# Ladme/groan_rs

Hardware: AMD Instinct MI355X
Metric: frames/sec RMSD-fit, 1e6 atoms triclinic, 1/2/4/8 GPUs; HBM GB/s vs peak (higher is better)
Workload: dtype f32 (fp64 accumulators)

## Files before the change

### groan_rs_amd/csrc/gr_api.hip

```cpp
#include <hip/hip_runtime.h>

#include <cmath>
#include <cstdio>
#include <cstdlib>
#include <cstring>
#include <map>
#include <string>
#include <vector>

#include "../../include/groan_hip.h"
#include "gr_batch.h"
#include "gr_buf.h"
#include "gr_workers.h"
#include "gr_container.h"
#include "gr_kernels.h"
#include "gr_hot.h"
#include "gr_resident.h"
#include "gr_small.h"
#include "gr_xtc.h"
#include "gr_shape.h"
#include "gr_xtc_dev.h"
#include "gr_xtc_enc_dev.h"
#include "gr_trr.h"
#include "gr_cellgrid.h"
// ... 394 lines not shown
    if (c->in_flight && slot < c->in_flight_s0 + c->in_flight_n && c->in_flight_s0 < slot + n)
        return fail(c, GR_E_INVALID_ARG, "upload into a slot of the batch in flight: call gr_rmsd_batch_end first (or use the other half of the double buffer)");
    return GR_OK;
}

struct SlotUse {
    gr_ctx *c; uint32_t first, n;
    bool quiet = false;
    SlotUse(gr_ctx *ctx, uint32_t first_slot, uint32_t count = 1) : c(ctx), first(first_slot), n(count) {
        for (uint32_t s = first; s < first + n && s < c->n_slots; ++s)
            if (c->upload_pending[s]) { (void)hipStreamWaitEvent(c->stream, c->ev_ready[s], 0); c->upload_pending[s] = 0; }
    }
    ~SlotUse() {
        if (quiet) return;
        const uint64_t gen = ++c->done_gen;
        (void)hipEventRecord(c->ev_done_ring[gen % 64], c->stream);
        for (uint32_t s = first; s < first + n && s < c->n_slots; ++s) c->slot_gen[s] = gen;
    }
};

static hipError_t sync_ingest(gr_ctx *c) {
    hipError_t e = hipStreamSynchronize(c->copy_stream);
    if (e == hipSuccess && c->unpack_stream) e = hipStreamSynchronize(c->unpack_stream);
    return e;
}
static int slot_box_wait(gr_ctx *c, uint32_t slot) {
    if (c->ev_ready[slot]) HIPCHK(c, hipEventSynchronize(c->ev_ready[slot]));
    else HIPCHK(c, hipEventCreateWithFlags(&c->ev_ready[slot], hipEventDisableTiming));
    return GR_OK;
}
void box_fill(gr_ctx *c, uint32_t slot, const float *box9) {
    GrBox &b = c->boxes_host[slot];
    if (!box9) {
        gr_box_setup(nullptr, &b);
        c->box_status[slot] = GR_E_NO_BOX; c->box9_set[slot] = 0;
    } else {
        const int ok = gr_box_setup(box9, &b);
        memcpy(&c->box9_host[9 * (size_t)slot], box9, 9 * sizeof(float));
        c->box9_set[slot] = 1;
        if (!ok) c->box_status[slot] = GR_E_ZERO_BOX;
        else if (b.ncand > GR_MAX_CAND) c->box_status[slot] = GR_E_UNSUPPORTED_BOX;
        else c->box_status[slot] = GR_OK;
    }
}
int set_box(gr_ctx *c, uint32_t slot, const float *box9, hipStream_t on = nullptr) {
    box_fill(c, slot, box9);
    HIPCHK(c, hipMemcpyAsync(c->boxes_dev + slot, &c->boxes_host[slot], sizeof(GrBox), hipMemcpyHostToDevice, on ? on : c->stream));
    return GR_OK;
}

int set_boxes_same(gr_ctx *c, uint32_t first_slot, uint32_t n, const float *box9, hipStream_t on = nullptr) {
    if (n == 0) return GR_OK;
    float keep[9];
    if (box9) memcpy(keep, box9, sizeof keep);
    box_fill(c, first_slot, box9 ? keep : nullptr);
    for (uint32_t f = 1; f < n; ++f) {
        const uint32_t s = first_slot + f;
        c->boxes_host[s] = c->boxes_host[first_slot];
        c->box_status[s] = c->box_status[first_slot]; c->box9_set[s] = c->box9_set[first_slot];
        if (box9) memcpy(&c->box9_host[9 * (size_t)s], keep, sizeof keep);
    }
    HIPCHK(c, hipMemcpyAsync(c->boxes_dev + first_slot, c->boxes_host + first_slot, (size_t)n * sizeof(GrBox), hipMemcpyHostToDevice, on ? on : c->stream));
    return GR_OK;
}

int ensure_staging(gr_ctx *c, float **buf) {
    if (*buf) return GR_OK;
    HIPCHK(c, hipMalloc(buf, c->frame_stride * sizeof(float)));
    HIPCHK(c, hipMemsetAsync(*buf, 0, c->frame_stride * sizeof(float), c->stream));
    HIPCHK(c, hipStreamSynchronize(c->stream));
    return GR_OK;
}
int untile_slot(gr_ctx *c, uint32_t slot) {
    int st = ensure_staging(c, &c->aos_dl); if (st) return st;
    const uint32_t ng = (uint32_t)(c->n_pad >> 2);
    k_untile<<<dim3((ng + 255) / 256), dim3(256), 0, c->stream>>>(c->frames + (size_t)slot * c->frame_stride, c->aos_dl, ng);
    HIPCHK(c, hipGetLastError());
    return GR_OK;
}

int ensure_event(gr_ctx *c, hipEvent_t *ev, bool timing) {
    if (*ev) return GR_OK;
    HIPCHK(c, timing ? hipEventCreate(ev) : hipEventCreateWithFlags(ev, hipEventDisableTiming));
    return GR_OK;
}
#define EVREC(ctx, ev, timing, stream) do { int s_ = ensure_event((ctx), &(ev), (timing)); if (s_) return s_; HIPCHK((ctx), hipEventRecord((ev), (stream))); } while (0)

int state_reset(gr_ctx *c, uint32_t n) {
    k_state_reset<<<dim3((n + 63) / 64), dim3(64), 0, c->stream>>>(c->state_dev, n);
    HIPCHK(c, hipGetLastError());
    return GR_OK;
}

int fetch_states(gr_ctx *c, uint32_t n) {
    HIPCHK(c, hipMemcpyAsync(c->state_host, c->state_dev, n * sizeof(GrFrameState), hipMemcpyDeviceToHost, c->stream));
    HIPCHK(c, hipStreamSynchronize(c->stream));
    return GR_OK;
}

int frame_status(gr_ctx *c, const GrFrameState &st) {
    if (st.status == GR_OK) return GR_OK;
    if (st.status == GR_E_NO_POSITION) return fail(c, GR_E_NO_POSITION, "atom has no position", st.err_index);
    if (st.status == GR_E_NO_MASS) return fail(c, GR_E_NO_MASS, "atom has no mass", st.err_index);
    return fail(c, st.status, "frame analysis failed");
}

static bool small_ok(const gr_ctx *c, const GrSel &sel) { return c->small_max != 0 && c->small_state != nullptr && sel.n <= c->small_max && !c->profile; }
static int small_wait(gr_ctx *c, uint32_t seq, uint32_t words = 1) {
    volatile uint32_t *w = c->small_flag;
    const auto t0 = std::chrono::steady_clock::now();
    for (uint32_t spins = 0; w[0] != seq || w[words - 1] != seq; ++spins) {
        if ((spins & 1023u) == 1023u && std::chrono::steady_clock::now() - t0 > std::chrono::milliseconds(20)) {
            c->small_sync_fallbacks++;
            HIPCHK(c, hipStreamSynchronize(c->stream));
            if (w[0] != seq || w[words - 1] != seq) return fail(c, GR_E_HIP, "a single-wave kernel ended without publishing its result");
            break;
        }
    }
    std::atomic_thread_fence(std::memory_order_acquire);
    c->small_calls++;
    return GR_OK;
}

static int res_next_epoch(gr_ctx *c, uint32_t *epoch) {
    if (++c->res_epoch == 0u) {
        HIPCHK(c, hipStreamSynchronize(c->stream));
        if (c->res_wgrec.get()) HIPCHK(c, hipMemset(c->res_wgrec.get(), 0, c->res_wgrec.cap() * sizeof(unsigned long long)));
        HIPCHK(c, hipMemset(c->res_rec, 0, (size_t)GR_MAX_BATCH * 16 * sizeof(unsigned long long)));
        HIPCHK(c, hipMemset(c->res_abort + 2, 0, 2 * sizeof(uint32_t)));
        c->res_epoch = 1u;
    }
    *epoch = c->res_epoch;
    return GR_OK;
}
static int res_wgrec_reserve(gr_ctx *c, size_t rec_words, hipStream_t S) {
    bool grew = false;
    HIPCHK(c, c->res_wgrec.reserve(rec_words, grbuf::exact, &grew));
    const hipError_t e = grew ? hipMemsetAsync(c->res_wgrec.get(), 0, rec_words * sizeof(unsigned long long), S) : hipSuccess;
    if (e != hipSuccess) c->res_wgrec.release();
    HIPCHK(c, e);
    return GR_OK;
}
static int res_test_no_start(gr_ctx *c, uint32_t epoch) {
    if (!c->res_test_no_start) return GR_OK;
    const unsigned long long two = 2ull | ((unsigned long long)epoch << 32);
    c->res_test_no_start = 0;
    HIPCHK(c, hipMemcpyAsync(c->res_abort + 2, &two, sizeof two, hipMemcpyHostToDevice, c->stream));
    HIPCHK(c, hipStreamSynchronize(c->stream));
    return GR_OK;
}
template <int MODE>
static int res_close(gr_ctx *c, uint32_t nb, const double *fit_partials, uint32_t nparts, double sum_w, uint32_t epoch, bool fresh, uint32_t *seq) {
    const uint32_t sq = c->res_seq + 1u;
    k_res_close<MODE><<<dim3(nb), dim3(64), 0, c->stream>>>(fit_partials, nparts, sum_w, c->state_dev, c->res_rec, epoch, fresh ? 1u : 0u, c->res_abort, c->res_closed + nb,
                                                        c->res_out_dev->st, c->res_out_dev->words, &c->res_out_dev->seq, sq);
    HIPCHK(c, hipGetLastError());
    c->res_seq = sq; c->res_closed += nb; *seq = sq;
    return GR_OK;
}
static int res_collect(gr_ctx *c, uint32_t seq, uint32_t nb, uint32_t epoch, bool *started) {
    volatile uint32_t *w = &c->res_out->seq;
    const auto t0 = std::chrono::steady_clock::now();
    for (uint32_t spins = 0; *w != seq; ++spins) {
        if ((spins & 1023u) == 1023u && std::chrono::steady_clock::now() - t0 > std::chrono::milliseconds(20)) {
            c->res_sync_fallbacks++;
            HIPCHK(c, hipStreamSynchronize(c->stream));
            if (*w != seq) return fail(c, GR_E_HIP, "the kernel behind the resident pass ended without publishing its results");
            break;
        }
    }
    std::atomic_thread_fence(std::memory_order_acquire);
    memcpy(c->state_host, c->res_out->st, (size_t)nb * sizeof(GrFrameState));
    memcpy(c->res_words_host, c->res_out->words, 12 * sizeof(uint32_t));
    for (int k = 0; k < 2; ++k) { const uint32_t v = c->res_words_host[8 + k]; c->res_words_host[8 + k] = v - c->res_late_seen[k]; c->res_late_seen[k] = v; }
    *started = c->res_words_host[2] == 1u && c->res_words_host[3] == epoch;
    if (!*started || c->res_words_host[0]) HIPCHK(c, hipStreamSynchronize(c->stream));
    return GR_OK;
}

int center_stage(gr_ctx *c, uint32_t first_slot, uint32_t nf, const GrSel &sel, int kind, int weighted,
                 int mass_first, int target, int only_status = 0) {
    if (small_ok(c, sel)) {
        k_center_small_stage<<<dim3(nf), dim3(64), 0, c->stream>>>(c->frames, c->frame_stride, first_slot, c->masses, sel, c->boxes_dev, kind, weighted, mass_first, target, c->state_dev, only_status);
        HIPCHK(c, hipGetLastError());
        return GR_OK;
    }
    uint32_t nch = chunks_for(sel);
    if (nf > 1 && nch >= 8) nch &= ~7u;
    const dim3 grid(nch, nf), wg(GR_WG);
    if (kind == 0) k_center_sums<0><<<grid, wg, 0, c->stream>>>(c->frames, c->frame_stride, first_slot, c->masses, sel, c->boxes_dev, c->state_dev, weighted, c->cen_partials, only_status);
    else if (kind == 1) k_center_sums<1><<<grid, wg, 0, c->stream>>>(c->frames, c->frame_stride, first_slot, c->masses, sel, c->boxes_dev, c->state_dev, weighted, c->cen_partials, only_status);
    else k_center_sums<2><<<grid, wg, 0, c->stream>>>(c->frames, c->frame_stride, first_slot, c->masses, sel, c->boxes_dev, c->state_dev, weighted, c->cen_partials, only_status);
    k_center_finalize<<<dim3(nf), dim3(GR_WG), 0, c->stream>>>(c->cen_partials, nch, c->boxes_dev, first_slot, kind, weighted, mass_first, target, sel.n, c->state_dev, only_status);
    HIPCHK(c, hipGetLastError());
    return GR_OK;
}

int pbc_center_stages(gr_ctx *c, uint32_t first_slot, uint32_t nf, const GrSel &sel, int weighted, int only_status = 0) {
    if (small_ok(c, sel) && only_status == 0) {
        k_center_small_pbc<<<dim3(nf), dim3(64), 0, c->stream>>>(c->frames, c->frame_stride, first_slot, c->masses, sel, c->boxes_dev, weighted, c->state_dev);
        HIPCHK(c, hipGetLastError());
        return GR_OK;
    }
    int st = center_stage(c, first_slot, nf, sel, 1, 0, 0, 0, only_status);
    if (st != GR_OK) return st;
    return center_stage(c, first_slot, nf, sel, 2, weighted, 0, 1, only_status);
}

static bool center_onepass_ok(const gr_ctx *c, const GrSel &sel) {
    return c->com_onepass_min != 0 && (sel.contiguous || sel.masked) && sel.n >= c->com_onepass_min && c->two_pass;
}
static int pbc_center_onepass(gr_ctx *c, uint32_t s0, uint32_t nb, const GrSel &sel, int weighted) {
    GrPlanDev plan; memset(&plan, 0, sizeof plan);
    plan.w_is_mass = weighted ? 1u : 0u;
    plan.n = sel.n; plan.sw = 1.0;
    const uint32_t nch = batch_chunks(c, sel, nb);
    if (sel.masked) {
        k_sums_pk<true, false, true><<<dim3(nch, nb), dim3(GR_WG), 0, c->stream>>>(c->frames, c->frame_stride, s0, c->masses, sel, c->boxes_dev, plan, c->acc_partials,
                                                                                   c->fuse ? c->fuse_cnt : nullptr, c->fuse ? c->state_dev : nullptr);
        if (!c->fuse) k_rmsd_finalize_lite<true><<<dim3(nb), dim3(64), 0, c->stream>>>(c->acc_partials, nch, c->frames, c->frame_stride, s0, sel, c->boxes_dev, plan, c->state_dev);
    } else if (c->fuse) {
        k_sums_pk<true><<<dim3(nch, nb), dim3(GR_WG), 0, c->stream>>>(c->frames, c->frame_stride, s0, c->masses, sel, c->boxes_dev, plan, c->acc_partials, c->fuse_cnt, c->state_dev);
    } else {
        k_sums_pk<true><<<dim3(nch, nb), dim3(GR_WG), 0, c->stream>>>(c->frames, c->frame_stride, s0, c->masses, sel, c->boxes_dev, plan, c->acc_partials, nullptr, nullptr);
        k_rmsd_finalize_lite<true><<<dim3(nb), dim3(64), 0, c->stream>>>(c->acc_partials, nch, c->frames, c->frame_stride, s0, sel, c->boxes_dev, plan, c->state_dev);
    }
    HIPCHK(c, hipGetLastError());
    return GR_OK;
}
static int center_redo_fallbacks(gr_ctx *c, uint32_t s0, uint32_t nb, const GrSel &sel, int weighted, std::vector<GrFrameState> &res) {
    uint32_t n_fb = 0, n_amb = 0;
    for (uint32_t f = 0; f < nb; ++f) { n_fb += c->state_host[f].status == GR_ST_FALLBACK; n_amb += c->state_host[f].status == GR_ST_AMBIG; }
    if (n_fb || n_amb) {
        c->center_fallbacks += n_fb + n_amb;
        int st = GR_OK;
        if (n_amb) { st = center_stage(c, s0, nb, sel, 1, 0, 0, 0, GR_ST_AMBIG); if (st) return st; }
        if (n_fb) { st = pbc_center_stages(c, s0, nb, sel, weighted, GR_ST_FALLBACK); if (st) return st; }
        st = fetch_states(c, nb); if (st) return st;
    }
    res.assign(c->state_host, c->state_host + nb);
    return GR_OK;
}

}

static int gr_abi_guard() { return GR_E_HIP; }

extern "C" {

const char *gr_version(void) { return "groan_hip 0.1.0 (gfx950)"; }

const char *gr_status_string(int s) try {
    switch (s) {
    case GR_OK: return "ok";
    case GR_E_NO_BOX: return "simulation box does not exist";
    case GR_E_NOT_ORTHOGONAL: return "simulation box is not orthogonal";
    case GR_E_ZERO_BOX: return "box length is zero or negative";
    case GR_E_EMPTY_GROUP: return "group is empty";
    case GR_E_INCONSISTENT_GROUP: return "group has a different number of atoms in reference and target";
    case GR_E_NO_POSITION: return "atom has undefined position";
    case GR_E_NO_MASS: return "atom has undefined mass";
    case GR_E_GROUP_NOT_FOUND: return "group does not exist";
    case GR_E_OUT_OF_RANGE: return "atom index out of range";
    case GR_E_INVALID_ARG: return "invalid argument";
    case GR_E_GROUP_EXISTS: return "group already existed and was overwritten";
    case GR_E_HIP: return "HIP runtime error";
    case GR_E_NO_DEVICE: return "no usable HIP device";
    case GR_E_UNSUPPORTED_BOX: return "box too skewed for the minimum-image table";
    case GR_E_IO: return "file could not be opened or read";
    case GR_E_FORMAT: return "not a valid xtc file";
    case GR_E_INVALID_NAME: return "invalid group name";
    case GR_E_EMPTY_CHAIN: return "no acceptor and no donor atoms detected for chain";
    case GR_E_NONEXISTENT_CHAIN: return "chain does not exist";
    case GR_E_DUPLICATE_PAIR: return "pair of chains requested multiple times";
    case GR_E_UNUSED_CHAIN: return "not all chains are used";
    case GR_E_INVALID_BOND: return "invalid bond";
    case GR_E_INVALID_SPAN: return "invalid span of the grid map";
    case GR_E_INVALID_TILE: return "invalid grid tile";
    default: return "unknown status";
    }
} catch (...) { return nullptr; }

int gr_device_count(int *count) try {
    int n = 0;
    if (hipGetDeviceCount(&n) != hipSuccess) { if (count) *count = 0; return GR_E_NO_DEVICE; }
    if (count) *count = n;
    return n > 0 ? GR_OK : GR_E_NO_DEVICE;
} catch (...) { return gr_abi_guard(); }

gr_ctx *gr_ctx_create(int device, uint64_t n_atoms, uint32_t n_slots, int *status) try {
    int dummy; if (!status) status = &dummy;
    int ndev = 0;
    if (hipGetDeviceCount(&ndev) != hipSuccess || ndev <= 0 || device < 0 || device >= ndev) { *status = GR_E_NO_DEVICE; return nullptr; }
    if (n_atoms == 0 || n_atoms > 0xFFFFFFF0ull || n_slots == 0) { *status = GR_E_INVALID_ARG; return nullptr; }
    if (hipSetDevice(device) != hipSuccess) { *status = GR_E_NO_DEVICE; return nullptr; }
    gr_ctx *c = new gr_ctx();
    c->device = device; c->n = n_atoms; c->n_pad = (n_atoms + 255) & ~255ull; c->n_slots = n_slots;
    c->frame_stride = (size_t)c->n_pad * 3;
    bool ok = true;
    ok = ok && hipStreamCreateWithFlags(&c->stream, hipStreamNonBlocking) == hipSuccess;
    ok = ok && hipStreamCreateWithFlags(&c->copy_stream, hipStreamNonBlocking) == hipSuccess;
    for (int k = 0; k < 64; ++k) ok = ok && hipEventCreateWithFlags(&c->ev_done_ring[k], hipEventDisableTiming) == hipSuccess;
    c->ev_ready.assign(n_slots, nullptr); c->upload_pending.assign(n_slots, 0); c->slot_gen.assign(n_slots, 0);
    ok = ok && hipMalloc(&c->fuse_cnt, 2 * GR_MAX_BATCH * sizeof(uint32_t)) == hipSuccess;
    ok = ok && hipMemset(c->fuse_cnt, 0, 2 * GR_MAX_BATCH * sizeof(uint32_t)) == hipSuccess;
    { hipDeviceProp_t prop; if (hipGetDeviceProperties(&prop, device) == hipSuccess) c->n_cus = (uint32_t)prop.multiProcessorCount; }
    ok = ok && hipMalloc(&c->frames, (size_t)n_slots * c->frame_stride * sizeof(float)) == hipSuccess;
    ok = ok && hipMalloc(&c->masses, c->n_pad * sizeof(float)) == hipSuccess;
// ... 2625 lines not shown
```

### groan_rs_amd/csrc/gr_resident.h

```cpp
#pragma once
#include <type_traits>
#include "gr_hot.h"

struct GrResShape {
    static constexpr int LANES = 512, WAVES = LANES / 64;
#ifndef GR_RES_K
#define GR_RES_K 6
#endif
    static constexpr int K = GR_RES_K;
    static constexpr int R = 8;
    static constexpr int PARK_F4 = K * 3 * LANES;
    static constexpr int WSUM_F = R * WAVES * 32;
#ifdef GR_EXP_TIMELINE
    static constexpr int TL_BYTES = 128 * 4 * 8;
#else
    static constexpr int TL_BYTES = 0;
#endif
    static constexpr int LDS_BYTES = PARK_F4 * 16 + WSUM_F * 4 + R * WAVES * 8 + 3 * R * 4 + 2 * WAVES * 4 + TL_BYTES;
    static constexpr int REC_PER_WAVE = 256 / WAVES, LANES_PER_REC = 64 / REC_PER_WAVE, WORDS_PER_LANE = 32 / LANES_PER_REC;
};
#ifndef GR_RES_SLEEP
#define GR_RES_SLEEP 2
#endif
#ifndef GR_RES_BAL
// ... 792 lines not shown
            }
        } else if (status == 0) {
            GrResRot T;
            T.r00 = rec.r00; T.r10 = rec.r10; T.r20 = rec.r20; T.r01 = rec.r01; T.r11 = rec.r11; T.r21 = rec.r21;
            T.r02 = rec.r02; T.r12 = rec.r12; T.r22 = rec.r22;
            if (V) {
                const float t0x = rec.t0x, t0y = rec.t0y, t0z = rec.t0z;
                T.sx = T.sy = T.sz = 0.f;
                fit_group_v(GA, ra, T, t0x, t0y, t0z, oa, rs);
                if (GB.valid) fit_group_v(GB, rb, T, t0x, t0y, t0z, ob, rs);
            } else {
                T.sx = rec.sx; T.sy = rec.sy; T.sz = rec.sz;
                const GrBox *boxp = boxes + first_slot + kf(j);
                gr_res_fit_group<WMASS>(GA, ra.r0, ra.r1, ra.r2, T, B, boxp, cx, cy, cz, oa.r0, oa.r1, oa.r2, rs);
                if (GB.valid) gr_res_fit_group<WMASS>(GB, rb.r0, rb.r1, rb.r2, T, B, boxp, cx, cy, cz, ob.r0, ob.r1, ob.r2, rs);
            }
        }
        {
#ifdef GR_EXP_NOSTORE
            const __amdgpu_buffer_rsrc_t out = gr_buf_rsrc(frames + (size_t)(first_slot + kf(j)) * frame_stride, 0u);
#else
            const __amdgpu_buffer_rsrc_t out = gr_buf_rsrc(frames + (size_t)(first_slot + kf(j)) * frame_stride, status == 0 ? slot_bytes : 0u);
#endif
            gr_buf_store_stream(out, offA, oa.r0); gr_buf_store_stream(out, offA + 1024u, oa.r1); gr_buf_store_stream(out, offA + 2048u, oa.r2);
            gr_buf_store_stream(out, offB, ob.r0); gr_buf_store_stream(out, offB + 1024u, ob.r1); gr_buf_store_stream(out, offB + 2048u, ob.r2);
        }
        n_fitted = j + 1u;
        if (MODE == 1) return;
        const float wtot = gr_wave_allsum_f32(rs);
        if (lane == 0) fit_partials[((size_t)kf(j) * ctl.wgs_frame + wg) * WAVES + wave] = (double)wtot;
    };

    Landing L0, L1;
    L0.a.r0 = L0.a.r1 = L0.a.r2 = L0.b.r0 = L0.b.r1 = L0.b.r2 = zero4; L0.gx = L0.gy = L0.gz = 0.f;
    L1 = L0;
    Rows Q0, Q1, Q2, Q3, Q4, Q5;
    Q0.r0 = Q0.r1 = Q0.r2 = zero4; Q1 = Q0; Q2 = Q0; Q3 = Q0; Q4 = Q0; Q5 = Q0;
    unsigned long long rv = 0ull;
    gate(0);
    if (n_turns) request(0, L0);
    const uint32_t n_iter = n_turns + K;
    const GrBoxU B0 = gr_box_uniform(boxes + first_slot);
    auto lds_put = [&](uint32_t slot, const Rows &rw) { park[(slot * 3 + 0) * LANES + tid] = rw.r0; park[(slot * 3 + 1) * LANES + tid] = rw.r1; park[(slot * 3 + 2) * LANES + tid] = rw.r2; };
    auto lds_get = [&](uint32_t slot) { Rows rw; rw.r0 = park[(slot * 3 + 0) * LANES + tid]; rw.r1 = park[(slot * 3 + 1) * LANES + tid]; rw.r2 = park[(slot * 3 + 2) * LANES + tid]; return rw; };
    auto step_sums_first = [&](uint32_t i, Landing &cur, Landing &nxt) {
        rv = request_rec(i >= K && i < n_iter ? i - K : 0u);
#ifdef GR_EXP_NOLOAD
        if (i < 2) request(i + 1, nxt);
#else
        GR_STEP_STAMP(6);
        gate(i + 1);
        GR_STEP_STAMP(0);
        request(i + 1, nxt);
#endif
        balance(i);
        const GrBoxU Bf = UBOX ? B0 : gr_box_uniform(boxes + first_slot + kf(i >= K ? i - K : 0u));
        const GrBoxU Bs = UBOX ? B0 : gr_box_uniform(boxes + first_slot + kf(i < n_turns ? i : 0u));
        Rows va = cur.a, vb = cur.b;
        const uint32_t ps = i % K;
        GR_STEP_STAMP(1);
        if (i < n_turns) { if constexpr (MODE == 1) sums_cen(i, cur, Bs); else sums(i, cur, Bs, va, vb); }
#if GR_RES_LATE_COMBINE
        if (i == n_turns && n_turns > 0u && claim(n_turns - 1u)) { if constexpr (MODE == 1) combine_cen(n_turns - 1u); else combine_rmsd(n_turns - 1u); }
#endif
        GR_STEP_STAMP(3);
        if (i >= K) {
            Rows qb;
            if (ps == 0u) { qb = Q0; asm volatile("; set 0 out"); } else if (ps == 1u) { qb = Q1; asm volatile("; set 1 out"); } else if (ps == 2u) { qb = Q2; asm volatile("; set 2 out"); }
            else if (ps == 3u) { qb = Q3; asm volatile("; set 3 out"); } else if (ps == 4u) { qb = Q4; asm volatile("; set 4 out"); } else { qb = Q5; asm volatile("; set 5 out"); }
            fit(i - K, rv, lds_get(ps), qb, Bf);
            if (bail) return;
        }
        GR_STEP_STAMP(5);
        if (i < n_turns) {
            lds_put(ps, va);
            if (ps == 0u) { Q0 = vb; asm volatile("; set 0 in"); } else if (ps == 1u) { Q1 = vb; asm volatile("; set 1 in"); } else if (ps == 2u) { Q2 = vb; asm volatile("; set 2 in"); }
            else if (ps == 3u) { Q3 = vb; asm volatile("; set 3 in"); } else if (ps == 4u) { Q4 = vb; asm volatile("; set 4 in"); } else { Q5 = vb; asm volatile("; set 5 in"); }
        }
    };
    auto step_fit_first = [&](uint32_t i, Landing &cur, Landing &nxt) {
#ifdef GR_EXP_NOLOAD
        if (i < 2) request(i + 1, nxt);
#elif !defined(GR_EXP_LATE_REQUEST)
        gate(i + 1);
        request(i + 1, nxt);
#endif
        balance(i);
        const GrBoxU Bf = UBOX ? B0 : gr_box_uniform(boxes + first_slot + kf(i >= K ? i - K : 0u));
        const GrBoxU Bs = UBOX ? B0 : gr_box_uniform(boxes + first_slot + kf(i < n_turns ? i : 0u));
        Rows va = cur.a, vb = cur.b;
        const uint32_t ps = i % K;
        if (i >= K) {
            Rows qb;
            if (ps == 0u) { qb = Q0; asm volatile("; set 0 out"); } else if (ps == 1u) { qb = Q1; asm volatile("; set 1 out"); } else if (ps == 2u) { qb = Q2; asm volatile("; set 2 out"); }
            else if (ps == 3u) { qb = Q3; asm volatile("; set 3 out"); } else if (ps == 4u) { qb = Q4; asm volatile("; set 4 out"); } else { qb = Q5; asm volatile("; set 5 out"); }
            fit(i - K, rv, lds_get(ps), qb, Bf);
            if (bail) return;
        }
        rv = request_rec(i + 1 >= K && i + 1 < n_iter ? i + 1 - K : 0u);
#ifdef GR_EXP_LATE_REQUEST
        request(i + 1, nxt);
#endif
        if (i < n_turns) {
            if (MODE == 1) sums_cen(i, cur, Bs);
            else if (V) sums(i, cur, Bs, va, vb);
            lds_put(ps, va);
            if (ps == 0u) { Q0 = vb; asm volatile("; set 0 in"); } else if (ps == 1u) { Q1 = vb; asm volatile("; set 1 in"); } else if (ps == 2u) { Q2 = vb; asm volatile("; set 2 in"); }
            else if (ps == 3u) { Q3 = vb; asm volatile("; set 3 in"); } else if (ps == 4u) { Q4 = vb; asm volatile("; set 4 in"); } else { Q5 = vb; asm volatile("; set 5 in"); }
            if (!V && MODE != 1) sums(i, cur, Bs, va, vb);
        }
#if GR_RES_LATE_COMBINE
        if (i == n_turns && n_turns > 0u && claim(n_turns - 1u)) { if constexpr (MODE == 1) combine_cen(n_turns - 1u); else combine_rmsd(n_turns - 1u); }
#endif
    };
    auto step = [&](uint32_t i, Landing &cur, Landing &nxt) { if constexpr (FL) step_sums_first(i, cur, nxt); else step_fit_first(i, cur, nxt); };
    for (uint32_t i = 0; i < n_iter && !bail; i += 2) {
        step(i, L0, L1);
        if (!bail && i + 1 < n_iter) step(i + 1, L1, L0);
    }
    if (lane == 0) {
        ctl.progress[wg_all * WAVES + wave] = n_fitted;
        (void)__hip_atomic_fetch_max(reinterpret_cast<unsigned long long *>(ctl.abort + 6), (unsigned long long)wall_clock64(), __ATOMIC_RELAXED, __HIP_MEMORY_SCOPE_AGENT);
        if (n_late) (void)__hip_atomic_fetch_add(ctl.abort + 8, n_late, __ATOMIC_RELAXED, __HIP_MEMORY_SCOPE_AGENT);
        if (n_waited) (void)__hip_atomic_fetch_add(ctl.abort + 9, n_waited, __ATOMIC_RELAXED, __HIP_MEMORY_SCOPE_AGENT);
#ifdef GR_EXP_STEPTIME
        if (ctl.dbg) {
            unsigned long long *o = ctl.dbg + (size_t)(wg_all * WAVES + wave) * 4u;
            unsigned long long tot = 0; for (int k = 0; k < 7; ++k) tot += st_acc[k];
            o[0] = st_acc[4]; o[1] = st_acc[7] | (st_combines << 32);
            o[2] = (__builtin_amdgcn_s_getreg((20 << 0) | (0 << 6) | (3 << 11)) & 7u) | (simd_of[wave] << 8);
            o[3] = tot;
        }
        if ((wg_all == 0u || wg_all == ctl.n_stream / 2u) && (wave == 0u || wave == 5u)) {
            unsigned long long *o = reinterpret_cast<unsigned long long *>(ctl.abort + 16) + ((wg_all ? 2u : 0u) + (wave ? 1u : 0u)) * 8u;
            for (int k = 0; k < 8; ++k) o[k] = st_acc[k];
        }
#endif
        if (clk_wave) {
            const unsigned long long dc = (unsigned long long)clock64() - clk_c0, dw = (unsigned long long)wall_clock64() - clk_w0;
            gr_st_agent(ctl.abort + 10, (uint32_t)(dc >> 8)); gr_st_agent(ctl.abort + 11, (uint32_t)(dw >> 8));
        }
    }
#ifdef GR_EXP_TIMELINE
    if (tl_wg && wave == 0 && !bail) {
        for (uint32_t t = (n_turns > 128u ? n_turns - 128u : 0u) + lane; t < n_turns; t += 64u) {
            const size_t f = kf(t);
            ctl.tl[f * 8 + 0] = tls[(t & 127u) * 4u + 0u];
            ctl.tl[f * 8 + 6] = tls[(t & 127u) * 4u + 1u] | (tls[(t & 127u) * 4u + 2u] << 48);
        }
    }
#endif
}

template <int MODE>
__global__ __launch_bounds__(64) void k_res_close(const double *__restrict__ fit_partials, uint32_t nparts, double sum_w, GrFrameState *state,
                                                  const unsigned long long *__restrict__ rec, uint32_t epoch, uint32_t fresh_states, uint32_t *ctl_words,
                                                  uint32_t done_target, GrFrameState *out_states, uint32_t *out_words, uint32_t *out_seq, uint32_t seq) {
    constexpr uint32_t NW = sizeof(GrFrameState) / 4u, W_RMSD = offsetof(GrFrameState, rmsd) / 4u, W_STATUS = offsetof(GrFrameState, status) / 4u;
    static_assert(sizeof(GrFrameState) % 4u == 0 && NW <= 64u, "a frame state is exported by one wave, a word per lane");
    const uint32_t frame = blockIdx.x, lane = threadIdx.x;
    uint32_t *sw = reinterpret_cast<uint32_t *>(state + frame);
    uint32_t w = 0u;
    if (fresh_states && (uint32_t)(gr_ld_agent(rec + (size_t)frame * 16u) >> 32) != epoch) {
        GrFrameState z = {};
        z.err_index = GR_NOIDX; z.status = GR_ST_ABORTED;
        if (lane < NW) { w = reinterpret_cast<const uint32_t *>(&z)[lane]; sw[lane] = w; }
    } else if (lane < NW) w = sw[lane];
    const int status = __shfl((int)w, (int)W_STATUS, 64);
    if (MODE == 0 && status == 0) {
        double s0 = 0.0, s1 = 0.0, s2 = 0.0, s3 = 0.0;
        const double *p = fit_partials + (size_t)frame * nparts;
        uint32_t k = lane;
        for (; k + 192 < nparts; k += 256) { s0 += p[k]; s1 += p[k + 64]; s2 += p[k + 128]; s3 += p[k + 192]; }
        for (; k < nparts; k += 64) s0 += p[k];
        const double s = gr_wave_sum((s0 + s1) + (s2 + s3));
        float r = 0.0f;
        if (lane == 0) { r = (float)sqrt(fmax(s, 0.0) / sum_w); state[frame].rmsd = r; }
        r = __shfl(r, 0, 64);
        if (lane == W_RMSD) w = __float_as_uint(r);
    }
    if (lane < NW) reinterpret_cast<uint32_t *>(out_states + frame)[lane] = w;
    __threadfence_system();
    uint32_t n = 0u;
    if (lane == 0) n = __hip_atomic_fetch_add(ctl_words + 12, 1u, __ATOMIC_ACQ_REL, __HIP_MEMORY_SCOPE_AGENT) + 1u;
    n = (uint32_t)__builtin_amdgcn_readfirstlane((int)n);
    if (n != done_target) return;
    if (lane < 12u) out_words[lane] = gr_ld_agent(ctl_words + lane);
    __threadfence_system();
    if (lane == 0) __hip_atomic_store(out_seq, seq, __ATOMIC_RELEASE, __HIP_MEMORY_SCOPE_SYSTEM);
}
```

Before: 142,700.

## Pack eight frames per close workgroup and export states from the last block

```diff
diff --git a/groan_rs_amd/csrc/gr_api.hip b/groan_rs_amd/csrc/gr_api.hip
--- a/groan_rs_amd/csrc/gr_api.hip
+++ b/groan_rs_amd/csrc/gr_api.hip
@@ -570,8 +570,10 @@
 template <int MODE>
 static int res_close(gr_ctx *c, uint32_t nb, const double *fit_partials, uint32_t nparts, double sum_w, uint32_t epoch, bool fresh, uint32_t *seq) {
     const uint32_t sq = c->res_seq + 1u;
-    k_res_close<MODE><<<dim3(nb), dim3(64), 0, c->stream>>>(fit_partials, nparts, sum_w, c->state_dev, c->res_rec, epoch, fresh ? 1u : 0u, c->res_abort, c->res_closed + nb,
-                                                        c->res_out_dev->st, c->res_out_dev->words, &c->res_out_dev->seq, sq);
+    static_assert(GR_MAX_CHUNKS * GrResShape::WAVES <= 256u * GR_RES_CLOSE_TRIPS, "k_res_close has a frame's fit sums in flight at once");
+    constexpr uint32_t F = GR_RES_CLOSE_FRAMES;
+    k_res_close<MODE><<<dim3((nb + F - 1u) / F), dim3(64u * F), 0, c->stream>>>(fit_partials, nparts, sum_w, c->state_dev, nb, c->res_rec, epoch, fresh ? 1u : 0u, c->res_abort,
+                                                                            c->res_closed + nb, c->res_out_dev->st, c->res_out_dev->words, &c->res_out_dev->seq, sq);
     HIPCHK(c, hipGetLastError());
     c->res_seq = sq; c->res_closed += nb; *seq = sq;
     return GR_OK;
diff --git a/groan_rs_amd/csrc/gr_resident.h b/groan_rs_amd/csrc/gr_resident.h
--- a/groan_rs_amd/csrc/gr_resident.h
+++ b/groan_rs_amd/csrc/gr_resident.h
@@ -968,40 +968,82 @@
 #endif
 }
 
+constexpr uint32_t GR_RES_CLOSE_FRAMES = 8;
+constexpr uint32_t GR_RES_CLOSE_TRIPS = 8;
 template <int MODE>
-__global__ __launch_bounds__(64) void k_res_close(const double *__restrict__ fit_partials, uint32_t nparts, double sum_w, GrFrameState *state,
+__global__ __launch_bounds__(64 * GR_RES_CLOSE_FRAMES) void k_res_close(const double *__restrict__ fit_partials, uint32_t nparts, double sum_w, GrFrameState *state, uint32_t nb,
                                                   const unsigned long long *__restrict__ rec, uint32_t epoch, uint32_t fresh_states, uint32_t *ctl_words,
                                                   uint32_t done_target, GrFrameState *out_states, uint32_t *out_words, uint32_t *out_seq, uint32_t seq) {
-    constexpr uint32_t NW = sizeof(GrFrameState) / 4u, W_RMSD = offsetof(GrFrameState, rmsd) / 4u, W_STATUS = offsetof(GrFrameState, status) / 4u;
-    static_assert(sizeof(GrFrameState) % 4u == 0 && NW <= 64u, "a frame state is exported by one wave, a word per lane");
-    const uint32_t frame = blockIdx.x, lane = threadIdx.x;
-    uint32_t *sw = reinterpret_cast<uint32_t *>(state + frame);
-    uint32_t w = 0u;
-    if (fresh_states && (uint32_t)(gr_ld_agent(rec + (size_t)frame * 16u) >> 32) != epoch) {
-        GrFrameState z = {};
-        z.err_index = GR_NOIDX; z.status = GR_ST_ABORTED;
-        if (lane < NW) { w = reinterpret_cast<const uint32_t *>(&z)[lane]; sw[lane] = w; }
-    } else if (lane < NW) w = sw[lane];
-    const int status = __shfl((int)w, (int)W_STATUS, 64);
-    if (MODE == 0 && status == 0) {
-        double s0 = 0.0, s1 = 0.0, s2 = 0.0, s3 = 0.0;
-        const double *p = fit_partials + (size_t)frame * nparts;
-        uint32_t k = lane;
-        for (; k + 192 < nparts; k += 256) { s0 += p[k]; s1 += p[k + 64]; s2 += p[k + 128]; s3 += p[k + 192]; }
-        for (; k < nparts; k += 64) s0 += p[k];
-        const double s = gr_wave_sum((s0 + s1) + (s2 + s3));
-        float r = 0.0f;
-        if (lane == 0) { r = (float)sqrt(fmax(s, 0.0) / sum_w); state[frame].rmsd = r; }
-        r = __shfl(r, 0, 64);
-        if (lane == W_RMSD) w = __float_as_uint(r);
-    }
-    if (lane < NW) reinterpret_cast<uint32_t *>(out_states + frame)[lane] = w;
+    constexpr uint32_t F = GR_RES_CLOSE_FRAMES, T = GR_RES_CLOSE_TRIPS, NW = sizeof(GrFrameState) / 4u, W_STATUS = offsetof(GrFrameState, status) / 4u, W_ERR = offsetof(GrFrameState, err_index) / 4u;
+    static_assert(sizeof(GrFrameState) % 8u == 0 && F <= 16u, "states are copied 8 bytes at a time; a workgroup is at most 1 024 threads");
+    enum : uint32_t { KEEP = 0u, RMSD = 1u, ABORTED = 2u };
+    __shared__ uint32_t verdict[F], ticket;
+    __shared__ float rmsd[F];
+    const uint32_t wave = threadIdx.x >> 6, lane = threadIdx.x & 63u, frame0 = blockIdx.x * F, frame = frame0 + wave;
+    const uint32_t nfr = nb - frame0 < F ? nb - frame0 : F;
+    if (frame < nb) {
+        const unsigned long long rec0 = gr_ld_agent(rec + (size_t)frame * 16u);
+        const int status = state[frame].status;
+        uint32_t v = KEEP;
+        if constexpr (MODE == 0) {
+            const double *p = fit_partials + (size_t)frame * nparts;
+            const uint32_t last = nparts - 1u;
+            const uint32_t trips = nparts > lane + 192u ? (nparts - lane - 192u + 255u) / 256u : 0u;
+            const uint32_t trips0 = nparts > 192u ? (nparts - 192u + 255u) / 256u : 0u;
+            const uint32_t k_rest = lane + 256u * trips;
+            double s0 = 0.0, s1 = 0.0, s2 = 0.0, s3 = 0.0;
+            double rest[3];
+#pragma unroll
+            for (uint32_t j = 0; j < 3u; ++j) rest[j] = p[min(k_rest + 64u * j, last)];
+            auto rounds = [&](uint32_t t0) {
+                double a[T][4];
+#pragma unroll
+                for (uint32_t t = 0; t < T; ++t)
+#pragma unroll
+                    for (uint32_t c = 0; c < 4u; ++c) a[t][c] = p[min(lane + 256u * (t0 + t) + 64u * c, last)];
+#pragma unroll
+                for (uint32_t t = 0; t < T; ++t)
+                    if (t0 + t < trips) { s0 += a[t][0]; s1 += a[t][1]; s2 += a[t][2]; s3 += a[t][3]; }
+            };
+            rounds(0u);
+            for (uint32_t t0 = T; t0 < trips0; t0 += T) rounds(t0);
+#pragma unroll
+            for (uint32_t j = 0; j < 3u; ++j) if (k_rest + 64u * j < nparts) s0 += rest[j];
+            const double s = gr_wave_sum((s0 + s1) + (s2 + s3));
+            if (status == 0) { v = RMSD; if (lane == 0) rmsd[wave] = (float)sqrt(fmax(s, 0.0) / sum_w); }
+        }
+        if (fresh_states && (uint32_t)(rec0 >> 32) != epoch) v = ABORTED;
+        if (lane == 0) verdict[wave] = v;
+    }
+    __syncthreads();
+    if (wave == 0) {
+        const uint32_t v = lane < nfr ? verdict[lane] : KEEP;
+        if (v == RMSD) state[frame0 + lane].rmsd = rmsd[lane];
+        if (__any(v == ABORTED)) {
+            uint32_t *sw = reinterpret_cast<uint32_t *>(state + frame0);
+            for (uint32_t i = lane; i < nfr * NW; i += 64u)
+                if (verdict[i / NW] == ABORTED) sw[i] = i % NW == W_STATUS ? (uint32_t)GR_ST_ABORTED : i % NW == W_ERR ? GR_NOIDX : 0u;
+        }
+        if (lane == 0) ticket = __hip_atomic_fetch_add(ctl_words + 12, nfr, __ATOMIC_ACQ_REL, __HIP_MEMORY_SCOPE_AGENT) + nfr;
+    }
+    __syncthreads();
+    if (ticket != done_target) return;
+    __builtin_amdgcn_fence(__ATOMIC_ACQUIRE, "agent");
+    uint32_t word = 0u;
+    if (threadIdx.x < 12u) word = gr_ld_agent(ctl_words + threadIdx.x);
+    constexpr uint32_t U = 16u, NT = 64u * F;
+    const unsigned long long *src = reinterpret_cast<const unsigned long long *>(state);
+    unsigned long long *dst = reinterpret_cast<unsigned long long *>(out_states);
+    const uint32_t units = nb * (uint32_t)(sizeof(GrFrameState) / 8u);
+    for (uint32_t i0 = threadIdx.x; i0 < units; i0 += NT * U) {
+        unsigned long long x[U];
+#pragma unroll
+        for (uint32_t u = 0; u < U; ++u) x[u] = src[min(i0 + NT * u, units - 1u)];
+#pragma unroll
+        for (uint32_t u = 0; u < U; ++u) if (i0 + NT * u < units) dst[i0 + NT * u] = x[u];
+    }
+    if (threadIdx.x < 12u) out_words[threadIdx.x] = word;
     __threadfence_system();
-    uint32_t n = 0u;
-    if (lane == 0) n = __hip_atomic_fetch_add(ctl_words + 12, 1u, __ATOMIC_ACQ_REL, __HIP_MEMORY_SCOPE_AGENT) + 1u;
-    n = (uint32_t)__builtin_amdgcn_readfirstlane((int)n);
-    if (n != done_target) return;
-    if (lane < 12u) out_words[lane] = gr_ld_agent(ctl_words + lane);
-    __threadfence_system();
-    if (lane == 0) __hip_atomic_store(out_seq, seq, __ATOMIC_RELEASE, __HIP_MEMORY_SCOPE_SYSTEM);
+    __syncthreads();
+    if (threadIdx.x == 0) __hip_atomic_store(out_seq, seq, __ATOMIC_RELEASE, __HIP_MEMORY_SCOPE_SYSTEM);
 }
```

Result: no change. 142,500 (-0.2%).
